# david-jk/BigGAN-Tensorflow

Hardware: AMD Instinct MI355X
Metric: BigGAN-128 train-step images/sec (higher is better)
Workload: dtype bf16; 1 GPU; BigGAN-128 ch=96 bf16 (BASELINE config 3: global batch 256, 32/GPU over 8 GPUs); img_size=128, ch=96, per_gpu_batch=256, global_batch=256, da_policy=full, g_regularization=ortho_cosine, n_labels=0, gan_type=hinge, hip_graph=False, precision=bf16, parallelism=dp1

## Files before the change

### biggan-tensorflow_amd/csrc/igemm16.hip

```cpp
#include <stdlib.h>

#include "common.h"
#include "igemm.h"
#include "igemm16.h"
#include <type_traits>
#include "igemm_dev.h"

namespace bg {

typedef float f32x4_t __attribute__((ext_vector_type(4)));
typedef float f32x16_t __attribute__((ext_vector_type(16)));
typedef __bf16 bf16x8_t __attribute__((ext_vector_type(8)));
typedef short s16x4v __attribute__((ext_vector_type(4)));
typedef short s16x8v __attribute__((ext_vector_type(8)));
typedef __attribute__((address_space(3))) void lds_void_t;
typedef __attribute__((address_space(1))) const void gbl_void_t;
typedef __attribute__((address_space(3))) s16x4v lds_s16x4v;

__device__ uint4 g_zero_page[1024];

__device__ __forceinline__ void glds16(const void* src, unsigned char* lds_wave_base) {
    __builtin_amdgcn_global_load_lds((gbl_void_t*)src, (lds_void_t*)lds_wave_base, 16, 0, 0);
}

__device__ __forceinline__ void glds16_asm(const void* src, uint32_t lds_byte_addr) {
    unsigned keep;
    const uint32_t dst = __builtin_amdgcn_readfirstlane(lds_byte_addr);
    asm volatile("s_mov_b32 %0, m0\n\ts_mov_b32 m0, %2\n\ts_nop 0\n\tglobal_load_lds_dwordx4 %1, off\n\ts_mov_b32 m0, %0"
                 : "=&s"(keep)
                 : "v"(src), "s"(dst)
                 : "memory");
}

__device__ __forceinline__ uint32_t pack_bf16x2(float a, float b) {
    typedef __bf16 bf16x2_t __attribute__((ext_vector_type(2)));
    bf16x2_t v;
    v[0] = (__bf16)a;
    v[1] = (__bf16)b;
    return __builtin_bit_cast(uint32_t, v);
}
__device__ __forceinline__ float bf16_lo(uint32_t u) { return __builtin_bit_cast(float, u << 16); }
__device__ __forceinline__ float bf16_hi(uint32_t u) { return __builtin_bit_cast(float, u & 0xffff0000u); }

constexpr int NN16_BM = 128;
constexpr int NN16_TAPS = 4;
constexpr int NN16_RING_TAPS = 8;
constexpr int nn16_lds_bytes(int TN, int TAPS = NN16_TAPS) {
    const int stage = (NN16_BM + 32 * TN) * 128;
    const int epi = NN16_BM * (32 * TN + 4) * 4;
    const int tab = 2 * TAPS * NN16_BM * 4;
    return (2 * stage + tab > epi ? 2 * stage + tab : epi) + NN16_BM * 4 + 16;
}
constexpr int NN16_NOSRC = -(1 << 30);

template <int MODE>
__device__ __forceinline__ int64_t nn16_src_off(const Gather& g, const RowPos& r, int kh, int kw) {
    int h, w;
    if (MODE == GATHER_CONV) {
        h = conv_src(r.ho, kh, g.stride, g.pad, g.reflect, g.Hs);
        w = conv_src(r.wo, kw, g.stride, g.pad, g.reflect, g.Ws);
    } else {
        h = tconv_src_from_num(r.ho + g.pad - kh, g.stride, g.Hs);
        w = tconv_src_from_num(r.wo + g.pad - kw, g.stride, g.Ws);
    }
    const bool ok = r.valid && h >= 0 && w >= 0;
    const int pix = (r.b * g.Hs + h) * g.Ws + w;
    return ok ? (int64_t)pix * g.ld : (int64_t)-1;
}

constexpr int NN16_NOMIRROR = -(1 << 20);
__device__ __forceinline__ int nn16_mirror_pos(int o, int n, bool hi) {
    return o == 1 ? -1 : ((hi && o == n - 2) ? n : NN16_NOMIRROR);
}

template <int MODE, bool PM, bool RING = false>
__device__ __forceinline__ RowPos nn16_row(const NN16Params& p, int m, int ph, int pw) {
    RowPos r;
    if (PM) {
        r.valid = m < p.M;
        const int pos = m / p.g.Nb;
        r.b = m - pos * p.g.Nb;
        if (RING) {
            const int L = p.ring_lines, first = L * p.g.Wo;
            if (pos < first) {
                const int line = pos / p.g.Wo;
                r.ho = line == 0 ? 1 : p.g.Ho - 2;
                r.wo = pos - line * p.g.Wo;
            } else {
                const int per = p.g.Ho - L, q = pos - first;
                const int line = q / per, idx = q - line * per;
                r.wo = line == 0 ? 1 : p.g.Wo - 2;
                r.ho = idx == 0 ? 0 : ((L == 2 && idx > p.g.Ho - 4) ? p.g.Ho - 1 : idx + 1);
            }
            return r;
        }
        const int hq = pos / p.g.Wq;
        r.ho = hq * p.g.pstep + ph;
        r.wo = (pos - hq * p.g.Wq) * p.g.pstep + pw;
        return r;
    }
    if (MODE == GATHER_PLAIN || !p.pow2) return decompose_row<MODE>(p.g, m, p.M, ph, pw);
    r.valid = m < p.M;
    const int wq = m & (p.g.Wq - 1);
    const int t = m >> p.wq_shift;
    const int hq = t & (p.g.Hq - 1);
    r.b = t >> p.hq_shift;
    r.ho = hq * p.g.pstep + ph;
    r.wo = wq * p.g.pstep + pw;
    return r;
}

template <int TN, int MODE, bool PM, bool RING = false>
__global__ __launch_bounds__(256, 2) void nn16_kernel(const NN16Params p) {
    static_assert(!RING || (PM && MODE == GATHER_TCONV), "ring launches are position-major transposed gathers");
    constexpr int TAPS = RING ? NN16_RING_TAPS : NN16_TAPS;
    constexpr int LDS_BYTES = nn16_lds_bytes(TN, TAPS);
    typedef typename std::conditional<RING, uint64_t, unsigned>::type mask_t;
    constexpr int BM = NN16_BM, BN = 32 * TN;
    constexpr int JA = BM / 32, JB = BN / 32;
    constexpr int A_BYTES = BM * 128, STAGE = (BM + BN) * 128;
    extern __shared__ __attribute__((aligned(16))) unsigned char smem[];

    const int t = threadIdx.x;
    const int lane = t & 63, w = t >> 6;
    const int wm = w >> 1, wn = w & 1;
    const Gather& g = p.g;

    int tile_m, tile_n, bz = blockIdx.z;
    if (p.zfold > 0) {
        const int lin = xcd_remap(blockIdx.x, p.tiles_m * p.tiles_n * p.zfold);
        if (p.mfast) {
            tile_m = lin % p.tiles_m;
            const int r_ = lin / p.tiles_m;
            bz = r_ % p.zfold;
            tile_n = r_ / p.zfold;
        } else {
            bz = lin % p.zfold;
            const int tile = lin / p.zfold;
            tile_n = tile % p.tiles_n;
            tile_m = tile / p.tiles_n;
        }
    } else {
        const int tile = xcd_remap(blockIdx.x, p.tiles_m * p.tiles_n);
        if (p.mfast) {
            tile_m = tile % p.tiles_m;
            tile_n = tile / p.tiles_m;
        } else {
            tile_n = tile % p.tiles_n;
            tile_m = tile / p.tiles_n;
        }
    }
    const int m0 = tile_m * BM, n0 = tile_n * BN;
    const int zs = bz % p.splitk, zo = bz / p.splitk;

    int ph = 0, pw = 0;
    if (MODE == GATHER_TCONV) {
        ph = g.pstep - 1 - zo / g.pstep;
        pw = g.pstep - 1 - zo % g.pstep;
    }
    int kh0 = 0, kw0 = 0, kstep = 1, nkh = g.k, nkw = g.k;
    if (MODE == GATHER_TCONV && g.pstep > 1) {
        kstep = g.stride;
        kh0 = (ph + g.pad) % g.stride;
        kw0 = (pw + g.pad) % g.stride;
        nkh = (g.k - kh0 + g.stride - 1) / g.stride;
        nkw = (g.k - kw0 + g.stride - 1) / g.stride;
    }
    int nrh = 0, nrw = 0;
    if (RING) {
        nrh = nrw = g.k;
        nkh = nkw = 2 * g.k;
    }
    const int C8 = p.C >> 3;
    const int ntap = nkh * nkw;

    unsigned& s_any = *reinterpret_cast<unsigned*>(smem + LDS_BYTES - 16);
    if (PM) {
        if (t == 0) s_any = 0;
        __syncthreads();
    }
    unsigned any_local = 0;
    int* tabh = reinterpret_cast<int*>(smem + 2 * STAGE);
    int* tabw = tabh + TAPS * BM;
    for (int e = t; e < 2 * TAPS * BM; e += 256) {
        const int axis = e / (TAPS * BM), i = (e / BM) % TAPS, row = e % BM;
        const RowPos r = nn16_row<MODE, PM, RING>(p, m0 + row, ph, pw);
        int v = NN16_NOSRC;
        if (r.valid && i < (axis ? nkw : nkh)) {
            int kk = (axis ? kw0 : kh0) + i * kstep;
            int o = axis ? r.wo : r.ho;
            const int n = axis ? g.Ws : g.Hs;
            if (RING) {
                const int nr = axis ? nrw : nrh;
                if (i >= nr) {
                    kk = i - nr;
                    o = nn16_mirror_pos(o, axis ? g.Wo : g.Ho, p.ring_lines == 2);
                }
            }
            const int src = MODE == GATHER_CONV ? conv_src(o, kk, g.stride, g.pad, g.reflect, n)
                                                : (o == NN16_NOMIRROR ? -1 : tconv_src_from_num(o + g.pad - kk, g.stride, n));
            if (src >= 0) {
                v = axis ? src : (r.b * g.Hs + src) * g.Ws;
                any_local |= 1u << (axis * TAPS + i);
            }
        }
        tabh[e] = v;
    }
    if (PM && any_local) atomicOr(&s_any, any_local);
    unsigned* tabo = reinterpret_cast<unsigned*>(smem + LDS_BYTES - 16 - BM * 4);
    constexpr bool use_tabo = MODE == GATHER_TCONV || PM;
    if (use_tabo && t < BM) {
        const RowPos r = nn16_row<MODE, PM, RING>(p, m0 + t, ph, pw);
        tabo[t] = (r.valid && r.ho < g.Ho && r.wo < g.Wo) ? (unsigned)((r.b * g.Ho + r.ho) * g.Wo + r.wo) : 0xffffffffu;
    }

    const int cch = (lane & 7) ^ ((((w & 1) << 2) | (lane >> 4)) & 7);
    const int rsub = 8 * w + (lane >> 3);
    const unsigned char* abase = reinterpret_cast<const unsigned char*>(p.A);
    const unsigned char* bbase = reinterpret_cast<const unsigned char*>(p.B);
    const unsigned char* zero = reinterpret_cast<const unsigned char*>(g_zero_page);
    const unsigned ald2 = 2u * (unsigned)g.ld;
    const uint32_t lds0 = static_cast<uint32_t>(
        reinterpret_cast<uintptr_t>((__attribute__((address_space(3))) unsigned char*)smem));

    __syncthreads();
    mask_t tapmask = 0;
    if (PM) {
        const unsigned any = __builtin_amdgcn_readfirstlane(s_any);
        for (int i = 0; i < nkh; ++i)
            for (int j = 0; j < nkw; ++j)
                if (((any >> i) & (any >> (TAPS + j)) & 1u) != 0 && !(RING && i < nrh && j < nrw))
                    tapmask |= (mask_t)1 << (i * TAPS + j);
    }
    const int nsteps_all = ((PM ? __builtin_popcountll((uint64_t)tapmask) : ntap) * C8 + 7) >> 3;
    const int sps = (nsteps_all + p.splitk - 1) / p.splitk;
    const int it0 = zs * sps;
    const int nsteps = max(0, min(nsteps_all, it0 + sps) - it0);

    mask_t rem = tapmask;
    int tidx = 0, c8, ih = 0, iw = 0;
    {
        const int kk = it0 * 8 + cch;
        tidx = kk / C8;
        c8 = kk - tidx * C8;
        if (PM) {
            for (int i = 0; i < tidx && rem; ++i) rem &= rem - 1;
        } else {
            ih = tidx / nkw;
            iw = tidx - ih * nkw;
        }
    }
    const unsigned char* asrc[JA];
    const unsigned char* wsrc[JB];
    auto set_tap = [&]() {
        bool kvalid;
        if (PM) {
            kvalid = rem != 0;
            const int bit = kvalid ? __builtin_ctzll((uint64_t)rem) : 0;
            ih = bit / TAPS;
            iw = bit % TAPS;
        } else {
            kvalid = tidx < ntap;
        }
        const int* th = tabh + (ih & (TAPS - 1)) * BM + rsub;
        const int* tw = tabw + (iw & (TAPS - 1)) * BM + rsub;
#pragma unroll
        for (int j = 0; j < JA; ++j) {
            const int pix = th[32 * j] + tw[32 * j];
            asrc[j] = (kvalid & (pix >= 0)) ? abase + (uint64_t)(unsigned)pix * ald2 : zero;
        }
        const int kh = RING ? (ih >= nrh ? ih - nrh : ih) : kh0 + ih * kstep;
        const int kw = RING ? (iw >= nrw ? iw - nrw : iw) : kw0 + iw * kstep;
        const unsigned char* wt = bbase + 2 * (int64_t)(kh * g.k + kw) * p.tap_stride;
#pragma unroll
        for (int j = 0; j < JB; ++j) {
            const int n = n0 + 32 * j + rsub;
            wsrc[j] = (kvalid & (n < p.N)) ? wt + 2 * (uint64_t)((unsigned)n * (unsigned)p.C) : zero;
        }
    };
    set_tap();

    auto stage = [&](int buf) {
        const uint32_t sa = lds0 + buf * STAGE + (8 * w) * 128;
        const uint32_t sb = sa + A_BYTES;
        const unsigned cbyte = 16u * (unsigned)c8;
#pragma unroll
        for (int j = 0; j < JA; ++j) glds16_asm(asrc[j] + cbyte, sa + j * 32 * 128);
#pragma unroll
        for (int j = 0; j < JB; ++j) glds16_asm(wsrc[j] + cbyte, sb + j * 32 * 128);
        c8 += 8;
        if (c8 >= C8) {
            do {
                c8 -= C8;
                if (PM) {
                    rem &= rem - 1;
                } else {
                    ++tidx;
                    if (++iw == nkw) {
                        iw = 0;
                        ++ih;
                    }
                }
            } while (c8 >= C8);
            set_tap();
        }
    };

    f32x4_t acc[4][TN];
#pragma unroll
    for (int i = 0; i < 4; ++i)
#pragma unroll
        for (int j = 0; j < TN; ++j)
#pragma unroll
            for (int r = 0; r < 4; ++r) acc[i][j][r] = 0.f;

    const int fsw = (lane & 15) >> 1;
    const int a_row = (wm * 64 + (lane & 15)) * 128;
    const int b_row = A_BYTES + (wn * 16 * TN + (lane & 15)) * 128;
    int koff[2];
#pragma unroll
    for (int s2 = 0; s2 < 2; ++s2) koff[s2] = 16 * ((4 * s2 + (lane >> 4)) ^ fsw);

    if (nsteps > 0) stage(0);
    asm volatile("s_waitcnt vmcnt(0) lgkmcnt(0)" ::: "memory");
    __builtin_amdgcn_s_barrier();

    for (int it = 0; it < nsteps; ++it) {
        const int cur = it & 1;
        if (it + 1 < nsteps) stage(cur ^ 1);
        const unsigned char* sbuf = smem + cur * STAGE;
        bf16x8_t a[2][4], b[2][TN];
#pragma unroll
        for (int s2 = 0; s2 < 2; ++s2) {
#pragma unroll
            for (int i = 0; i < 4; ++i)
                a[s2][i] = *reinterpret_cast<const bf16x8_t*>(sbuf + a_row + i * 16 * 128 + koff[s2]);
#pragma unroll
            for (int j = 0; j < TN; ++j)
                b[s2][j] = *reinterpret_cast<const bf16x8_t*>(sbuf + b_row + j * 16 * 128 + koff[s2]);
        }
#pragma unroll
        for (int s2 = 0; s2 < 2; ++s2)
#pragma unroll
            for (int i = 0; i < 4; ++i)
#pragma unroll
                for (int j = 0; j < TN; ++j)
                    acc[i][j] = __builtin_amdgcn_mfma_f32_16x16x32_bf16(b[s2][j], a[s2][i], acc[i][j], 0, 0, 0);
        asm volatile("s_waitcnt vmcnt(0) lgkmcnt(0)" ::: "memory");
        __builtin_amdgcn_s_barrier();
    }

    constexpr int ELD = BN + 4;
    float* est = reinterpret_cast<float*>(smem);
    const bool partial = p.splitk > 1;
    const float alpha = (!partial && p.alpha) ? *p.alpha : 1.0f;
#pragma unroll
    for (int i = 0; i < 4; ++i)
#pragma unroll
        for (int j = 0; j < TN; ++j) {
            const int row = wm * 64 + 16 * i + (lane & 15);
            const int col = wn * 16 * TN + 16 * j + 4 * (lane >> 4);
            f32x4_t v = acc[i][j];
            v[0] *= alpha; v[1] *= alpha; v[2] *= alpha; v[3] *= alpha;
            *reinterpret_cast<f32x4_t*>(est + row * ELD + col) = v;
        }
    __syncthreads();
    constexpr int CPR = BN / 8;
    float* slab = partial ? p.slabs + (int64_t)zs * p.slab_stride : nullptr;
#pragma unroll
    for (int q = 0; q < BM * CPR / 256; ++q) {
        const int idx = t + 256 * q;
        const int row = idx / CPR, cc = idx - row * CPR;
        const int m = m0 + row, col = n0 + cc * 8;
        if (m >= p.M || col >= p.N) continue;
        int64_t ooff;
        if (use_tabo) {
            const unsigned op = tabo[row];
            if (op == 0xffffffffu) continue;
            ooff = (int64_t)op * p.out_ld + col;
        } else if (p.d2s_c) {
            int b, ho, wo;
            if (p.pow2) {
                wo = m & (g.Wo - 1);
                const int t2 = m >> p.wq_shift;
                ho = t2 & (g.Ho - 1);
                b = t2 >> p.hq_shift;
            } else {
                const int t2 = m / g.Wo;
                wo = m - t2 * g.Wo;
                b = t2 / g.Ho;
                ho = t2 - b * g.Ho;
            }
            const int sub = col / p.d2s_c, c = col - sub * p.d2s_c;
            ooff = (((int64_t)b * (2 * g.Ho) + 2 * ho + (sub >> 1)) * (2 * g.Wo) + 2 * wo + (sub & 1)) * p.d2s_c + c;
        } else {
            ooff = (int64_t)m * p.out_ld + col;
        }
        f32x4_t v0 = *reinterpret_cast<const f32x4_t*>(est + row * ELD + cc * 8);
        f32x4_t v1 = *reinterpret_cast<const f32x4_t*>(est + row * ELD + cc * 8 + 4);
        if (partial) {
            *reinterpret_cast<f32x4_t*>(slab + ooff) = v0;
            *reinterpret_cast<f32x4_t*>(slab + ooff + 4) = v1;
            continue;
        }
        if (p.bias) {
            const f32x4_t b0 = *reinterpret_cast<const f32x4_t*>(p.bias + col);
            const f32x4_t b1 = *reinterpret_cast<const f32x4_t*>(p.bias + col + 4);
            v0 += b0;
            v1 += b1;
        }
        if (p.out_f32) {
            float* o = reinterpret_cast<float*>(p.out) + ooff;
            if (p.accumulate) {
                v0 += *reinterpret_cast<const f32x4_t*>(o);
                v1 += *reinterpret_cast<const f32x4_t*>(o + 4);
            }
            *reinterpret_cast<f32x4_t*>(o) = v0;
            *reinterpret_cast<f32x4_t*>(o + 4) = v1;
        } else {
            __bf16* o = reinterpret_cast<__bf16*>(p.out) + ooff;
            if (p.accumulate) {
                const uint4 r = *reinterpret_cast<const uint4*>(o);
                v0[0] += bf16_lo(r.x); v0[1] += bf16_hi(r.x); v0[2] += bf16_lo(r.y); v0[3] += bf16_hi(r.y);
                v1[0] += bf16_lo(r.z); v1[1] += bf16_hi(r.z); v1[2] += bf16_lo(r.w); v1[3] += bf16_hi(r.w);
            }
            uint4 r;
            r.x = pack_bf16x2(v0[0], v0[1]);
            r.y = pack_bf16x2(v0[2], v0[3]);
            r.z = pack_bf16x2(v1[0], v1[1]);
            r.w = pack_bf16x2(v1[2], v1[3]);
            *reinterpret_cast<uint4*>(o) = r;
        }
    }
}

__global__ __launch_bounds__(256) void nn16_slab_reduce_kernel(const float* __restrict__ slabs, void* __restrict__ out,
                                                               const float* __restrict__ bias,
                                                               const float* __restrict__ alpha_dev, int64_t n8, int N,
                                                               int splitk, int64_t slab_stride, int accumulate,
                                                               int out_f32) {
    const float alpha = alpha_dev ? *alpha_dev : 1.0f;
    for (int64_t i = (int64_t)blockIdx.x * 256 + threadIdx.x; i < n8; i += (int64_t)gridDim.x * 256) {
        f32x4_t s0 = {0.f, 0.f, 0.f, 0.f}, s1 = s0;
        for (int z = 0; z < splitk; ++z) {
            const float* sp = slabs + (int64_t)z * slab_stride + i * 8;
            s0 += *reinterpret_cast<const f32x4_t*>(sp);
            s1 += *reinterpret_cast<const f32x4_t*>(sp + 4);
        }
        s0 *= alpha;
        s1 *= alpha;
        if (bias) {
            const int col = (int)((i * 8) % N);
            s0 += *reinterpret_cast<const f32x4_t*>(bias + col);
            s1 += *reinterpret_cast<const f32x4_t*>(bias + col + 4);
        }
        if (out_f32) {
            float* o = reinterpret_cast<float*>(out) + i * 8;
            if (accumulate) {
                s0 += *reinterpret_cast<const f32x4_t*>(o);
                s1 += *reinterpret_cast<const f32x4_t*>(o + 4);
            }
            *reinterpret_cast<f32x4_t*>(o) = s0;
            *reinterpret_cast<f32x4_t*>(o + 4) = s1;
        } else {
            __bf16* o = reinterpret_cast<__bf16*>(out) + i * 8;
            if (accumulate) {
                const uint4 r = *reinterpret_cast<const uint4*>(o);
                s0[0] += bf16_lo(r.x); s0[1] += bf16_hi(r.x); s0[2] += bf16_lo(r.y); s0[3] += bf16_hi(r.y);
                s1[0] += bf16_lo(r.z); s1[1] += bf16_hi(r.z); s1[2] += bf16_lo(r.w); s1[3] += bf16_hi(r.w);
            }
            uint4 r;
            r.x = pack_bf16x2(s0[0], s0[1]);
            r.y = pack_bf16x2(s0[2], s0[3]);
            r.z = pack_bf16x2(s1[0], s1[1]);
            r.w = pack_bf16x2(s1[2], s1[3]);
            *reinterpret_cast<uint4*>(o) = r;
        }
    }
}

constexpr int NH_T = 16;
constexpr int NH_LDS_MAX = 81920;
template <int NT> struct NHGeom {
    static constexpr int HW = NH_T + NT - 1;
    static constexpr int NPIX = HW * HW;
    static constexpr int A_ROUNDS = (NPIX * 8 + 63) / 64;
    static constexpr int A_INSTR = (A_ROUNDS + 7) / 8;
    static constexpr int A_BYTES = A_ROUNDS * 1024;
};
constexpr int nh_w_rounds(int NF) { return 32 * NF * 8 / 64; }
constexpr int nh_w_instr(int NF) { return (nh_w_rounds(NF) + 7) / 8; }
constexpr int NH_WS = 2;
template <int NT, int NF> constexpr int nn16h_lds_bytes() {
    const int ring = NHGeom<NT>::A_BYTES + NH_WS * nh_w_rounds(NF) * 1024;
    const int epi = 128 * (32 * NF + 4) * 4;
    return ring > epi ? ring : epi;
}

struct NHTile {
    int b, y0, x0, n0, ph, pw, phase, nph, tx, ty, tiles_x, tiles_y;
};
template <int NF, int THIN>
__device__ __forceinline__ void nn16h_epilogue(const NN16Params& p, const NHTile& tl, f32x4_t (&acc)[4][NF],
                                               unsigned char* smem) {
    constexpr int BN = 32 * NF;
    const Gather& g = p.g;
    const int t = threadIdx.x, lane = t & 63, w = t >> 6;
    const int wm = w >> 1, wn = w & 1;
    const int px = lane & 15, kb = lane >> 4;
    const int b = tl.b, y0 = tl.y0, x0 = tl.x0, n0 = tl.n0, ph = tl.ph, pw = tl.pw, phase = tl.phase, nph = tl.nph;
    const int tx = tl.tx, ty = tl.ty, tiles_x = tl.tiles_x, tiles_y = tl.tiles_y;
    constexpr int ELD = BN + 4;
    float* est = reinterpret_cast<float*>(smem);
    const float alpha = p.alpha ? *p.alpha : 1.0f;
    constexpr int CPR = BN / 8;
// ... 761 lines not shown
}

struct NN16Plan {
    int tn, splitk;
};

static int nn16_steps_min(const NN16Params& p, int mode) {
    int per_axis = p.g.k;
    if (mode == GATHER_TCONV && p.g.pstep > 1) per_axis = max(1, p.g.k / p.g.stride);
    return (per_axis * per_axis * (p.C >> 3) + 7) >> 3;
}

static double nn16_axis_fraction(const Gather& g, int mode, int nq, int n_src) {
    int64_t valid = 0, slots = 0;
    for (int ph = 0; ph < (mode == GATHER_TCONV ? g.pstep : 1); ++ph) {
        int k0 = 0, kstep = 1, nk = g.k;
        if (mode == GATHER_TCONV && g.pstep > 1) {
            kstep = g.stride;
            k0 = (ph + g.pad) % g.stride;
            nk = (g.k - k0 + g.stride - 1) / g.stride;
        }
        for (int q = 0; q < nq; ++q) {
            const int o = q * g.pstep + ph;
            for (int i = 0; i < nk; ++i) {
                const int kk = k0 + i * kstep;
                bool ok;
                if (mode == GATHER_CONV) {
                    const int src = o * g.stride + kk - g.pad;
                    ok = g.reflect || (src >= 0 && src < n_src);
                } else {
                    const int hn = o + g.pad - kk;
                    ok = hn >= 0 && hn % g.stride == 0 && hn / g.stride < n_src;
                }
                valid += ok;
            }
            slots += nk;
        }
    }
    return slots ? (double)valid / (double)slots : 1.0;
}

static double nn16_posmajor_fraction(const NN16Params& p, int mode) {
    const char* e = getenv("BG_NN16_POSMAJOR");
    if (e && atoi(e) == 0) return 1.0;
    const Gather& g = p.g;
    if (g.k <= 1 || g.Nb < 16 || g.Hq <= 0 || g.Wq <= 0 || (int64_t)g.Hq * g.Wq > 40 * 40) return 1.0;
    const double f = nn16_axis_fraction(g, mode, g.Hq, g.Hs) * nn16_axis_fraction(g, mode, g.Wq, g.Ws);
    return f < 0.9 ? f : 1.0;
}

static NN16Plan plan_nn16(const NN16Params& p, int mode, int zdim, bool allow_split) {
    static const int slots = getenv("BG_NN16_SLOTS") ? atoi(getenv("BG_NN16_SLOTS")) : 512;
    const int64_t tm = (p.M + NN16_BM - 1) / NN16_BM;
    int steps = nn16_steps_min(p, mode);
    const double pm = nn16_posmajor_fraction(p, mode);
    if (pm < 1.0) steps = max(1, (int)(steps * pm + 0.5));
    NN16Plan best{4, 1};
    double best_cost = 1e30;
    for (int tn = 4; tn >= 1; --tn) {
        const int bn = 32 * tn;
        const int64_t tiles = tm * ((p.N + bn - 1) / bn) * zdim;
        const double unit = 1.5 + tn;
        const int max_sk = allow_split ? (steps / 4 < 16 ? (steps / 4 < 1 ? 1 : steps / 4) : 16) : 1;
        for (int sk = 1; sk <= max_sk; ++sk) {
            const int64_t rounds = (tiles * sk + slots - 1) / slots;
            double cost = (double)rounds * ((steps + sk - 1) / sk + 2.0) * unit;
            if (sk > 1) cost += 6.0 * unit + 0.02 * sk * (double)tiles / slots * bn;
            if (cost < best_cost - 1e-9) {
                best_cost = cost;
                best = NN16Plan{tn, sk};
            }
        }
    }
    return best;
}

size_t nn16_workspace_bytes(const NN16Params& p, int mode, int zdim, int64_t out_elems) {
    const NN16Plan pl = plan_nn16(p, mode, zdim, true);
    return pl.splitk > 1 ? (size_t)pl.splitk * out_elems * sizeof(float) : 0;
}

static int nn16_mfast(const NN16Params& p, int tiles_m, int tiles_n);

template <int TN>
static int launch_nn16_ring_inst(const NN16Params& p, dim3 grid, hipStream_t s) {
    constexpr int lds = nn16_lds_bytes(TN, NN16_RING_TAPS);
    if (!lds_opt_in(reinterpret_cast<const void*>(&nn16_kernel<TN, GATHER_TCONV, true, true>), lds)) return BG_ERR_LAUNCH;
    hipLaunchKernelGGL((nn16_kernel<TN, GATHER_TCONV, true, true>), grid, dim3(256), lds, s, p);
    return BG_OK;
}

int launch_nn16_ring(NN16Params& p, hipStream_t s) {
    BG_REQUIRE(p.ring == 1 && (p.ring_lines == 1 || p.ring_lines == 2), "nn16 ring launch: ring = 1, ring_lines 1 or 2");
    BG_REQUIRE(p.g.k >= 1 && p.g.k <= NN16_RING_TAPS / 2 && p.g.Ho >= 4 && p.g.Wo >= 4 && p.accumulate == 1,
               "nn16 ring launch: kernel size %d / map %d x %d not supported", p.g.k, p.g.Ho, p.g.Wo);
    BG_REQUIRE(p.C % 8 == 0 && p.N % 8 == 0 && p.g.ld % 8 == 0 && p.out_ld % 8 == 0, "nn16 ring launch: channels %% 8");
    const int npos = p.ring_lines * p.g.Wo + p.ring_lines * (p.g.Ho - p.ring_lines);
    p.g.pstep = 1;
    p.g.Hq = 1;
    p.g.Wq = npos;
    p.M = p.g.Nb * npos;
    p.posmajor = 1;
    p.splitk = 1;
    p.slabs = nullptr;
    p.zfold = 0;
    p.pow2 = 0;
    int tn = 4, best = 1 << 30;
    for (int c = 4; c >= 1; --c) {
        const int padded = (p.N + 32 * c - 1) / (32 * c) * (32 * c);
        if (padded < best) { best = padded; tn = c; }
    }
    p.tiles_m = (p.M + NN16_BM - 1) / NN16_BM;
    p.tiles_n = (p.N + 32 * tn - 1) / (32 * tn);
    p.mfast = nn16_mfast(p, p.tiles_m, p.tiles_n);
    dim3 grid(p.tiles_m * p.tiles_n, 1, 1);
    int rc;
    switch (tn) {
        case 1: rc = launch_nn16_ring_inst<1>(p, grid, s); break;
        case 2: rc = launch_nn16_ring_inst<2>(p, grid, s); break;
        case 3: rc = launch_nn16_ring_inst<3>(p, grid, s); break;
        default: rc = launch_nn16_ring_inst<4>(p, grid, s); break;
    }
    if (rc) return rc;
    BG_LAUNCH_CHECK();
    return BG_OK;
}

template <int TN, int MODE, bool PM>
static int launch_nn16_inst(const NN16Params& p, dim3 grid, hipStream_t s) {
    constexpr int lds = nn16_lds_bytes(TN);
    if (!lds_opt_in(reinterpret_cast<const void*>(&nn16_kernel<TN, MODE, PM>), lds)) return BG_ERR_LAUNCH;
    prof_kernel("nn16_kernel<%d, %d, %s>", TN, MODE, PM ? "true" : "false");
    hipLaunchKernelGGL((nn16_kernel<TN, MODE, PM>), grid, dim3(256), lds, s, p);
    return BG_OK;
}

template <int MODE, bool PM>
static int launch_nn16_pm(const NN16Params& p, int tn, dim3 grid, hipStream_t s) {
    switch (tn) {
        case 1: return launch_nn16_inst<1, MODE, PM>(p, grid, s);
        case 2: return launch_nn16_inst<2, MODE, PM>(p, grid, s);
        case 3: return launch_nn16_inst<3, MODE, PM>(p, grid, s);
        default: return launch_nn16_inst<4, MODE, PM>(p, grid, s);
    }
}

template <int MODE>
static int launch_nn16_mode(const NN16Params& p, int tn, dim3 grid, hipStream_t s) {
    return p.posmajor ? launch_nn16_pm<MODE, true>(p, tn, grid, s) : launch_nn16_pm<MODE, false>(p, tn, grid, s);
}

static int nn16h_taps(const NN16Params& p, int mode, int zdim) {
    const char* e = getenv("BG_NN16_HALO");
    const int use = e ? atoi(e) : 1;
    static const int cmax = getenv("BG_NN16_HALO_CMAX") ? atoi(getenv("BG_NN16_HALO_CMAX")) : 4096;
    const Gather& g = p.g;
    if (!use || p.C > cmax || p.C % 32 || p.N % 8 || g.Hq < NH_T || g.Wq < NH_T || g.Hq % NH_T || g.Wq % NH_T) return 0;
    if (mode == GATHER_CONV) return (g.stride == 1 && g.k == 3 && g.pstep == 1 && zdim == 1) ? 3 : 0;
    if (g.reflect) return 0;
    if (g.stride == 1 && g.k == 3 && g.pstep == 1 && zdim == 1) return 3;
    if (g.stride == 2 && g.k == 4 && g.pstep == 2 && zdim == 4) return 2;
    if (g.stride == 2 && g.k == 3 && g.pad == 1 && g.pstep == 2 && zdim == 4) {
        const char* e3 = getenv("BG_NN16_HALO_K3S2");
        return (e3 && atoi(e3) == 1) ? 2 : 0;
    }
    return 0;
}

template <int NT, int NF, int MODE, int THIN = 0>
static int launch_nn16h_inst(const NN16Params& p, int blocks, hipStream_t s) {
    constexpr int lds = nn16h_lds_bytes<NT, NF>();
    if (!lds_opt_in(reinterpret_cast<const void*>(&nn16h_kernel<NT, NF, MODE, THIN>), lds)) return BG_ERR_LAUNCH;
    if (THIN) prof_kernel("nn16h_kernel<%d, %d, %d, d2s>", NT, NF, MODE);
    else prof_kernel("nn16h_kernel<%d, %d, %d>", NT, NF, MODE);
    hipLaunchKernelGGL((nn16h_kernel<NT, NF, MODE, THIN>), dim3(blocks), dim3(512), lds, s, p);
    return BG_OK;
}

template <int NT, int MODE>
static int launch_nn16h_nf(const NN16Params& p, int nf, int blocks, hipStream_t s) {
    switch (nf) {
        case 1: return launch_nn16h_inst<NT, 1, MODE>(p, blocks, s);
        case 2: return launch_nn16h_inst<NT, 2, MODE>(p, blocks, s);
        case 3: return launch_nn16h_inst<NT, 3, MODE>(p, blocks, s);
        default: return launch_nn16h_inst<NT, 4, MODE>(p, blocks, s);
    }
}

bool nn16h_d2s_ok(const NN16Params& p) {
    const char* e = getenv("BG_THIN_D2S");
    const int use = e ? atoi(e) : 1;
    const Gather& g = p.g;
    return use && p.N == 8 && p.out_ld == 8 && g.k == 3 && g.stride == 2 && g.pad == 1 && !g.reflect && p.C % 32 == 0 &&
           g.Hs % NH_T == 0 && g.Ws % NH_T == 0 && g.Ho == 2 * g.Hs && g.Wo == 2 * g.Ws && !p.bias && !p.stats_part;
}
int launch_nn16h_d2s(const NN16Params& plain, hipStream_t s) {
    BG_REQUIRE(nn16h_d2s_ok(plain), "nn16h depth-to-space form: unsupported geometry");
    NN16Params p = plain;
    Gather& g = p.g;
    g.Hq = g.Hs; g.Wq = g.Ws; g.pstep = 1; g.pad = 0; g.stride = 1;
    p.N = 32;
    p.splitk = 1; p.mfast = 0; p.ring = 0;
    const int64_t blocks = (int64_t)g.Nb * (g.Hq / NH_T) * (g.Wq / NH_T);
    BG_REQUIRE(blocks > 0 && blocks < (int64_t(1) << 31), "nn16h: grid out of range");
    if (const int rc = launch_nn16h_inst<2, 1, GATHER_CONV, 1>(p, (int)blocks, s)) return rc;
    BG_LAUNCH_CHECK();
    return BG_OK;
}

static int nn16_mfast(const NN16Params& p, int tiles_m, int tiles_n) {
    const char* e = getenv("BG_NN16_MFAST");
    if (!e) return 0;
    if (strcmp(e, "auto") != 0) return atoi(e) != 0;
    const double l2 = 3.0e6;
    const double a_bytes = 2.0 * p.g.Nb * (double)p.g.Hs * p.g.Ws * p.g.ld;
    const double w_bytes = 2.0 * p.g.k * p.g.k * (double)p.N * p.C;
    const double nfast = a_bytes + (w_bytes > l2 ? w_bytes * tiles_m : w_bytes);
    const double mfast = w_bytes + (a_bytes > l2 ? a_bytes * tiles_n : a_bytes);
    return mfast < nfast;
}

static int launch_nn16h(NN16Params& p, int mode, int ntaps, hipStream_t s) {
    int nf = 4, best = 1 << 30;
    for (int c = 4; c >= 1; --c) {
        const int padded = (p.N + 32 * c - 1) / (32 * c) * (32 * c);
        if (padded < best) { best = padded; nf = c; }
    }
    const Gather& g = p.g;
    const int64_t blocks = (int64_t)g.Nb * (g.Hq / NH_T) * (g.Wq / NH_T) * ((p.N + 32 * nf - 1) / (32 * nf)) *
                           (g.pstep * g.pstep);
    BG_REQUIRE(blocks > 0 && blocks < (int64_t(1) << 31), "nn16h: grid out of range");
    p.splitk = 1;
    p.mfast = nn16_mfast(p, g.Nb * (g.Hq / NH_T) * (g.Wq / NH_T), (p.N + 32 * nf - 1) / (32 * nf));
    int rc;
    if (mode == GATHER_CONV) rc = launch_nn16h_nf<3, GATHER_CONV>(p, nf, (int)blocks, s);
    else if (ntaps == 3) rc = launch_nn16h_nf<3, GATHER_TCONV>(p, nf, (int)blocks, s);
    else rc = launch_nn16h_nf<2, GATHER_TCONV>(p, nf, (int)blocks, s);
    if (rc) return rc;
    BG_LAUNCH_CHECK();
    return BG_OK;
}

bool nn16_d2s_ok(const NN16Params& p, int mode, int zdim) {
    const Gather& g = p.g;
    if (p.d2s_c <= 0 || p.d2s_c % 8 || p.N != 4 * p.d2s_c || p.C % 8 || mode != GATHER_CONV || zdim != 1 || g.stride != 1 ||
        g.pstep != 1 || g.Hq != g.Ho || g.Wq != g.Wo || p.stats_part || p.ring)
        return false;
    if ((int64_t)g.Nb * g.Ho * g.Wo * 4 >= (int64_t(1) << 31)) return false;
    if (nn16h_taps(p, mode, zdim)) return true;
    if (nn16_posmajor_fraction(p, mode) < 1.0) return false;
    return plan_nn16(p, mode, zdim, true).splitk == 1;
}

int64_t nn16_stats_rows(const NN16Params& p, int mode, int zdim) {
    if (p.C % 8 || p.N % 8 || !nn16h_taps(p, mode, zdim)) return 0;
    return 2 * (int64_t)p.g.Nb * (p.g.Hq / NH_T) * (p.g.Wq / NH_T) * (p.g.pstep * p.g.pstep);
}

int launch_nn16(NN16Params& p, int mode, int zdim, int64_t out_elems, void* ws, size_t ws_bytes, hipStream_t s) {
    BG_REQUIRE(p.C % 8 == 0 && p.N % 8 == 0 && p.g.ld % 8 == 0 && p.out_ld % 8 == 0,
               "bf16-resident conv: channel counts must be multiples of 8 (C=%d N=%d)", p.C, p.N);
    BG_REQUIRE((reinterpret_cast<uintptr_t>(p.A) & 15) == 0 && (reinterpret_cast<uintptr_t>(p.B) & 15) == 0 &&
                   (reinterpret_cast<uintptr_t>(p.out) & 15) == 0,
               "bf16-resident conv: tensors must be 16-byte aligned");
    BG_REQUIRE(p.g.k >= 1 && p.g.k <= NN16_TAPS && p.C <= 8192 && p.g.stride >= 1 && p.g.stride <= 2,
               "bf16-resident conv: kernel size %d / stride %d / %d channels not supported", p.g.k, p.g.stride, p.C);
    BG_REQUIRE((int64_t)p.g.Nb * p.g.Hs * p.g.Ws < (int64_t(1) << 30) && (int64_t)p.g.Nb * p.g.Ho * p.g.Wo < (int64_t(1) << 31),
               "bf16-resident conv: more than 2^30 source / 2^31 output pixels");
    BG_REQUIRE(p.d2s_c == 0 || (nn16_d2s_ok(p, mode, zdim) && ws == nullptr),
               "bf16-resident conv: this launch has no depth-to-space store (bg_conv2d_fwd_d2s_supported)");
    if (const int ntaps = nn16h_taps(p, mode, zdim)) return launch_nn16h(p, mode, ntaps, s);
    BG_REQUIRE(p.stats_part == nullptr, "bf16-resident conv: fused statistics need the halo-tile form (nn16_stats_rows)");
    NN16Plan pl = plan_nn16(p, mode, zdim, ws != nullptr);
    if (pl.splitk > 1 && ws_bytes < (size_t)pl.splitk * out_elems * sizeof(float)) pl.splitk = 1;
    p.splitk = pl.splitk;
    p.slabs = reinterpret_cast<float*>(ws);
    p.slab_stride = out_elems;
    const int bn = 32 * pl.tn;
    p.tiles_m = (p.M + NN16_BM - 1) / NN16_BM;
    p.tiles_n = (p.N + bn - 1) / bn;
    p.pow2 = 0;
    if (p.g.Wq > 0 && p.g.Hq > 0 && (p.g.Wq & (p.g.Wq - 1)) == 0 && (p.g.Hq & (p.g.Hq - 1)) == 0) {
        p.pow2 = 1;
        p.wq_shift = __builtin_ctz(p.g.Wq);
        p.hq_shift = __builtin_ctz(p.g.Hq);
    }
    p.posmajor = nn16_posmajor_fraction(p, mode) < 1.0;
    p.mfast = nn16_mfast(p, p.tiles_m, p.tiles_n);
    dim3 grid(p.tiles_m * p.tiles_n, 1, zdim * p.splitk);
    p.zfold = 0;
    if (mode == GATHER_TCONV && zdim > 1 && p.splitk == 1 && p.g.k % p.g.stride == 0) {
        p.zfold = zdim;
        grid = dim3(p.tiles_m * p.tiles_n * zdim, 1, 1);
    }
    int rc;
    if (mode == GATHER_CONV)
        rc = launch_nn16_mode<GATHER_CONV>(p, pl.tn, grid, s);
    else
        rc = launch_nn16_mode<GATHER_TCONV>(p, pl.tn, grid, s);
    if (rc) return rc;
    BG_LAUNCH_CHECK();
    if (pl.splitk > 1) {
        const int64_t n8 = out_elems / 8;
        int blocks = (int)((n8 + 255) / 256);
        if (blocks > 2048) blocks = 2048;
        hipLaunchKernelGGL(nn16_slab_reduce_kernel, dim3(blocks), dim3(256), 0, s, p.slabs, p.out, p.bias, p.alpha, n8,
                           p.N, pl.splitk, out_elems, p.accumulate, p.out_f32);
        BG_LAUNCH_CHECK();
    }
    return BG_OK;
}

static void plan_tn16(TN16Params& p) {
    const int64_t tiles = (int64_t)((p.Mf + 127) / 128) * ((p.Cb + 127) / 128);
    static const int want = getenv("BG_TN16_WANT") ? atoi(getenv("BG_TN16_WANT")) : 1024;
    int sk = (int)(want / tiles);
    const int max_sk = (p.M + 4 * TN16_BK - 1) / (4 * TN16_BK);
    if (sk > max_sk) sk = max_sk;
    if (sk < 1) sk = 1;
    if (sk > 512) sk = 512;
    int rps = (p.M + sk - 1) / sk;
    rps = (rps + TN16_BK - 1) / TN16_BK * TN16_BK;
    p.splitk = (p.M + rps - 1) / rps;
    p.rows_per_split = rps;
}

static int tn16x_nbi(const TN16Params& p) {
    const char* e = getenv("BG_TN16X_NBI");
    if (!e || atoi(e) != 2) return 1;
    return (p.Cb >= 512 && p.Cb % 256 == 0 && p.Mf >= 256) ? 2 : 1;
}

static bool plan_tn16x(const TN16Params& p, int* sk_out, int* rps_out) {
    static const int use_wide = getenv("BG_TN16_WIDE") ? atoi(getenv("BG_TN16_WIDE")) : 1;
    if (!use_wide || p.Mf <= 128 || p.M < 8 * TN16_BK) return false;
    if (p.g.k > 0 && (p.g.Wq <= 0 || p.g.Hq <= 0 || (p.g.Wq & (p.g.Wq - 1)) || (p.g.Hq & (p.g.Hq - 1)))) return false;
    const int nbi = tn16x_nbi(p);
    const int tm = (p.Mf + 255) / 256, tn = (p.Cb + 128 * nbi - 1) / (128 * nbi);
    static const int wantx0 = getenv("BG_TN16X_WANT") ? atoi(getenv("BG_TN16X_WANT")) : 512;
    const int wantx = nbi == 2 ? wantx0 / 2 : wantx0;
    int sk = wantx / (tm * tn);
    const int max_sk = (p.M + 4 * TN16_BK - 1) / (4 * TN16_BK);
    if (sk > max_sk) sk = max_sk;
    if (sk < 1) sk = 1;
    if (sk > 512) sk = 512;
    int rps = (p.M + sk - 1) / sk;
    rps = (rps + TN16_BK - 1) / TN16_BK * TN16_BK;
    *sk_out = (p.M + rps - 1) / rps;
    *rps_out = rps;
    return true;
}

size_t tn16_workspace_bytes(const TN16Params& p0) {
    TN16Params p = p0;
    plan_tn16(p);
    int sk = p.splitk, skx = 1, rps = 0;
    if (plan_tn16x(p0, &skx, &rps) && skx > sk) sk = skx;
    return sk > 1 ? (size_t)sk * p.Mf * p.Cb * sizeof(float) : 0;
}

int launch_tn16(TN16Params& p, int mode, float* final_out, void* ws, size_t ws_bytes, hipStream_t s) {
    BG_REQUIRE(p.Ca % 8 == 0 && p.Cb % 8 == 0 && p.g.ld % 8 == 0 && p.b_ld % 8 == 0,
               "bf16-resident wgrad: channel counts must be multiples of 8 (Ca=%d Cb=%d)", p.Ca, p.Cb);
    BG_REQUIRE((reinterpret_cast<uintptr_t>(p.A) & 15) == 0 && (reinterpret_cast<uintptr_t>(p.Bv) & 15) == 0,
               "bf16-resident wgrad: tensors must be 16-byte aligned");
    plan_tn16(p);
    const int64_t total = (int64_t)p.Mf * p.Cb;
    if (p.splitk > 1 && (ws == nullptr || ws_bytes < (size_t)p.splitk * total * sizeof(float) || p.out_ld != p.Cb)) {
        p.splitk = 1;
        p.rows_per_split = (p.M + TN16_BK - 1) / TN16_BK * TN16_BK;
    }
    if (p.splitk > 1) {
        p.out = reinterpret_cast<float*>(ws);
        p.slab_stride = total;
    } else {
        p.out = final_out;
        p.slab_stride = 0;
    }
    p.tiles_m = (p.Mf + 127) / 128;
    p.tiles_n = (p.Cb + 127) / 128;
    p.pow2 = 0;
    if (mode != GATHER_PLAIN && (p.g.Wq & (p.g.Wq - 1)) == 0 && (p.g.Hq & (p.g.Hq - 1)) == 0) {
// ... 77 lines not shown
```

Measured before the change: 2673 images/sec.

## Add 3-slot LDS ring pipeline and 8-wave wide-tile form to nn16 conv

Adds a pipelined variant of the bf16 implicit-GEMM conv kernel. It uses a 3-slot LDS ring with half-width K steps (4 chunks), int16 column tables, and a partitioned epilogue, so loads for step k+2 overlap the MFMAs of step k. A wide 256-row, 8-wave form is chosen by default for small-channel, non-position-major launches with enough blocks, while the ring form is opt-in via an environment variable. The aim is better latency hiding and occupancy, at the cost of more barriers per K and changed tile shapes.

Result: faster. 2720 images/sec, median of 6 (+1.8%).

```diff
diff --git a/biggan-tensorflow_amd/csrc/igemm16.hip b/biggan-tensorflow_amd/csrc/igemm16.hip
--- a/biggan-tensorflow_amd/csrc/igemm16.hip
+++ b/biggan-tensorflow_amd/csrc/igemm16.hip
@@ -50,6 +50,10 @@
     const int epi = NN16_BM * (32 * TN + 4) * 4;
     const int tab = 2 * TAPS * NN16_BM * 4;
     return (2 * stage + tab > epi ? 2 * stage + tab : epi) + NN16_BM * 4 + 16;
+}
+constexpr int nn16_pipe_lds_bytes(int TN, int WM, int TAPS = NN16_TAPS) {
+    const int bm = 64 * WM;
+    return 3 * (bm + 32 * TN) * 64 + TAPS * bm * (4 + 2) + bm * 4 + 16;
 }
 constexpr int NN16_NOSRC = -(1 << 30);
 
@@ -110,19 +114,31 @@
     return r;
 }
 
-template <int TN, int MODE, bool PM, bool RING = false>
-__global__ __launch_bounds__(256, 2) void nn16_kernel(const NN16Params p) {
+template <int TN, int MODE, bool PM, bool RING = false, int SLOTS = 2, int WM = 2>
+__global__ __launch_bounds__(128 * WM, SLOTS == 2 ? 2 : (WM == 4 ? 4 : 3)) void nn16_kernel(const NN16Params p) {
     static_assert(!RING || (PM && MODE == GATHER_TCONV), "ring launches are position-major transposed gathers");
+    static_assert((SLOTS == 2 && WM == 2) || (SLOTS == 3 && (WM == 2 || WM == 4)), "two stages, or a 3-slot ring on 4 / 8 waves");
+    constexpr bool PIPE = SLOTS == 3;
     constexpr int TAPS = RING ? NN16_RING_TAPS : NN16_TAPS;
-    constexpr int LDS_BYTES = nn16_lds_bytes(TN, TAPS);
+    constexpr int LDS_BYTES = PIPE ? nn16_pipe_lds_bytes(TN, WM, TAPS) : nn16_lds_bytes(TN, TAPS);
     typedef typename std::conditional<RING, uint64_t, unsigned>::type mask_t;
-    constexpr int BM = NN16_BM, BN = 32 * TN;
-    constexpr int JA = BM / 32, JB = BN / 32;
-    constexpr int A_BYTES = BM * 128, STAGE = (BM + BN) * 128;
+    typedef typename std::conditional<PIPE, int16_t, int>::type tabw_t;
+    constexpr int BM = 64 * WM, BN = 32 * TN, NTHR = 128 * WM, NWV = 2 * WM;
+    constexpr int CPS = PIPE ? 4 : 8;
+    constexpr int ROWB = 16 * CPS;
+    constexpr int RSTR = PIPE ? 16 * NWV : 32;
+    constexpr int JA = BM / RSTR, JB = PIPE ? (BN / 16 + NWV - 1) / NWV : BN / 32;
+    constexpr int A_BYTES = BM * ROWB, STAGE = (BM + BN) * ROWB;
+    static_assert(BM == NN16_BM || PIPE, "the two-stage form has 128-row tiles");
+    static_assert(A_BYTES % 1024 == 0 && STAGE % 1024 == 0 && (RSTR * ROWB) % 1024 == 0,
+                  "every LDS-DMA destination is 1 KB aligned");
+    static_assert(!PIPE || 64 * (BN + 4) * 4 <= SLOTS * STAGE, "a 64-row part of the epilogue fits in front of the tables");
+    static_assert(!PIPE || RING || LDS_BYTES * (WM == 4 ? 2 : 3) <= 160 * 1024, "ring forms: 3 (8 waves: 2) blocks per CU");
+    static_assert(!PIPE || LDS_BYTES * 2 <= 160 * 1024, "mirrored-tap ring launches: 2 blocks per CU");
     extern __shared__ __attribute__((aligned(16))) unsigned char smem[];
 
     const int t = threadIdx.x;
-    const int lane = t & 63, w = t >> 6;
+    const int lane = t & 63, w = PIPE ? __builtin_amdgcn_readfirstlane(t >> 6) : t >> 6;
     const int wm = w >> 1, wn = w & 1;
     const Gather& g = p.g;
 
@@ -180,9 +196,9 @@
         __syncthreads();
     }
     unsigned any_local = 0;
-    int* tabh = reinterpret_cast<int*>(smem + 2 * STAGE);
-    int* tabw = tabh + TAPS * BM;
-    for (int e = t; e < 2 * TAPS * BM; e += 256) {
+    int* tabh = reinterpret_cast<int*>(smem + SLOTS * STAGE);
+    tabw_t* tabw = reinterpret_cast<tabw_t*>(tabh + TAPS * BM);
+    for (int e = t; e < 2 * TAPS * BM; e += NTHR) {
         const int axis = e / (TAPS * BM), i = (e / BM) % TAPS, row = e % BM;
         const RowPos r = nn16_row<MODE, PM, RING>(p, m0 + row, ph, pw);
         int v = NN16_NOSRC;
@@ -204,7 +220,8 @@
                 any_local |= 1u << (axis * TAPS + i);
             }
         }
-        tabh[e] = v;
+        if (PIPE && axis) tabw[e - TAPS * BM] = (tabw_t)(v < 0 ? -1 : v);
+        else tabh[e] = v;
     }
     if (PM && any_local) atomicOr(&s_any, any_local);
     unsigned* tabo = reinterpret_cast<unsigned*>(smem + LDS_BYTES - 16 - BM * 4);
@@ -214,8 +231,10 @@
         tabo[t] = (r.valid && r.ho < g.Ho && r.wo < g.Wo) ? (unsigned)((r.b * g.Ho + r.ho) * g.Wo + r.wo) : 0xffffffffu;
     }
 
-    const int cch = (lane & 7) ^ ((((w & 1) << 2) | (lane >> 4)) & 7);
-    const int rsub = 8 * w + (lane >> 3);
+    const int cch = PIPE ? (lane & 3) ^ ((lane >> 3) & 2) : (lane & 7) ^ ((((w & 1) << 2) | (lane >> 4)) & 7);
+    const int rsub = PIPE ? 16 * w + (lane >> 2) : 8 * w + (lane >> 3);
+    constexpr int NB_HI = JB, NB_LO = (BN / 16) / NWV;
+    const int nbw = (PIPE && NB_HI != NB_LO) ? (BN / 16 - w + NWV - 1) / NWV : JB;
     const unsigned char* abase = reinterpret_cast<const unsigned char*>(p.A);
     const unsigned char* bbase = reinterpret_cast<const unsigned char*>(p.B);
     const unsigned char* zero = reinterpret_cast<const unsigned char*>(g_zero_page);
@@ -263,10 +282,12 @@
             kvalid = tidx < ntap;
         }
         const int* th = tabh + (ih & (TAPS - 1)) * BM + rsub;
-        const int* tw = tabw + (iw & (TAPS - 1)) * BM + rsub;
+        const tabw_t* tw = tabw + (iw & (TAPS - 1)) * BM + rsub;
 #pragma unroll
         for (int j = 0; j < JA; ++j) {
-            const int pix = th[32 * j] + tw[32 * j];
+            int col = tw[RSTR * j];
+            if (PIPE) col = col < 0 ? NN16_NOSRC : col;
+            const int pix = th[RSTR * j] + col;
             asrc[j] = (kvalid & (pix >= 0)) ? abase + (uint64_t)(unsigned)pix * ald2 : zero;
         }
         const int kh = RING ? (ih >= nrh ? ih - nrh : ih) : kh0 + ih * kstep;
@@ -274,21 +295,13 @@
         const unsigned char* wt = bbase + 2 * (int64_t)(kh * g.k + kw) * p.tap_stride;
 #pragma unroll
         for (int j = 0; j < JB; ++j) {
-            const int n = n0 + 32 * j + rsub;
+            const int n = n0 + RSTR * j + rsub;
             wsrc[j] = (kvalid & (n < p.N)) ? wt + 2 * (uint64_t)((unsigned)n * (unsigned)p.C) : zero;
         }
     };
     set_tap();
-
-    auto stage = [&](int buf) {
-        const uint32_t sa = lds0 + buf * STAGE + (8 * w) * 128;
-        const uint32_t sb = sa + A_BYTES;
-        const unsigned cbyte = 16u * (unsigned)c8;
-#pragma unroll
-        for (int j = 0; j < JA; ++j) glds16_asm(asrc[j] + cbyte, sa + j * 32 * 128);
-#pragma unroll
-        for (int j = 0; j < JB; ++j) glds16_asm(wsrc[j] + cbyte, sb + j * 32 * 128);
-        c8 += 8;
+    auto advance = [&]() {
+        c8 += CPS;
         if (c8 >= C8) {
             do {
                 c8 -= C8;
@@ -306,6 +319,18 @@
         }
     };
 
+    auto stage = [&](int buf) {
+        const uint32_t sa = lds0 + buf * STAGE + w * 1024;
+        const uint32_t sb = sa + A_BYTES;
+        const unsigned cbyte = 16u * (unsigned)c8;
+#pragma unroll
+        for (int j = 0; j < JA; ++j) glds16_asm(asrc[j] + cbyte, sa + j * RSTR * ROWB);
+#pragma unroll
+        for (int j = 0; j < JB; ++j)
+            if (!PIPE || j < nbw) glds16_asm(wsrc[j] + cbyte, sb + j * RSTR * ROWB);
+        advance();
+    };
+
     f32x4_t acc[4][TN];
 #pragma unroll
     for (int i = 0; i < 4; ++i)
@@ -314,6 +339,40 @@
 #pragma unroll
             for (int r = 0; r < 4; ++r) acc[i][j][r] = 0.f;
 
+    if constexpr (PIPE) {
+        const int frag = (lane & 15) * ROWB + 16 * ((lane >> 4) ^ (((lane & 15) >> 1) & 2));
+        const unsigned char* a_ad = smem + wm * 64 * ROWB + frag;
+        const unsigned char* b_ad = smem + A_BYTES + wn * 16 * TN * ROWB + frag;
+        const int nst = 2 * nsteps;
+        if (nst > 0) stage(0);
+        if (nst > 1) stage(1);
+        auto kstep = [&](int it, auto slot_c) {
+            constexpr int SLOT = decltype(slot_c)::value;
+            if (it + 1 < nst) {
+                if (NB_HI == NB_LO || nbw == NB_HI) asm volatile("s_waitcnt vmcnt(%0) lgkmcnt(0)" ::"n"(JA + NB_HI) : "memory");
+                else asm volatile("s_waitcnt vmcnt(%0) lgkmcnt(0)" ::"n"(JA + NB_LO) : "memory");
+            } else
+                asm volatile("s_waitcnt vmcnt(0) lgkmcnt(0)" ::: "memory");
+            __builtin_amdgcn_s_barrier();
+            if (it + 2 < nst) stage((SLOT + 2) % 3);
+            bf16x8_t a[4], b[TN];
+#pragma unroll
+            for (int i = 0; i < 4; ++i) a[i] = *reinterpret_cast<const bf16x8_t*>(a_ad + SLOT * STAGE + i * 16 * ROWB);
+#pragma unroll
+            for (int j = 0; j < TN; ++j) b[j] = *reinterpret_cast<const bf16x8_t*>(b_ad + SLOT * STAGE + j * 16 * ROWB);
+#pragma unroll
+            for (int i = 0; i < 4; ++i)
+#pragma unroll
+                for (int j = 0; j < TN; ++j)
+                    acc[i][j] = __builtin_amdgcn_mfma_f32_16x16x32_bf16(b[j], a[i], acc[i][j], 0, 0, 0);
+        };
+        for (int it = 0; it < nst; it += 3) {
+            kstep(it, std::integral_constant<int, 0>());
+            if (it + 1 < nst) kstep(it + 1, std::integral_constant<int, 1>());
+            if (it + 2 < nst) kstep(it + 2, std::integral_constant<int, 2>());
+        }
+        __syncthreads();
+    } else {
     const int fsw = (lane & 15) >> 1;
     const int a_row = (wm * 64 + (lane & 15)) * 128;
     const int b_row = A_BYTES + (wn * 16 * TN + (lane & 15)) * 128;
@@ -349,28 +408,37 @@
         asm volatile("s_waitcnt vmcnt(0) lgkmcnt(0)" ::: "memory");
         __builtin_amdgcn_s_barrier();
     }
-
+    }
+
+    constexpr int PARTS = PIPE ? WM : 1, PR = BM / PARTS;
     constexpr int ELD = BN + 4;
     float* est = reinterpret_cast<float*>(smem);
     const bool partial = p.splitk > 1;
     const float alpha = (!partial && p.alpha) ? *p.alpha : 1.0f;
-#pragma unroll
-    for (int i = 0; i < 4; ++i)
-#pragma unroll
-        for (int j = 0; j < TN; ++j) {
-            const int row = wm * 64 + 16 * i + (lane & 15);
-            const int col = wn * 16 * TN + 16 * j + 4 * (lane >> 4);
-            f32x4_t v = acc[i][j];
-            v[0] *= alpha; v[1] *= alpha; v[2] *= alpha; v[3] *= alpha;
-            *reinterpret_cast<f32x4_t*>(est + row * ELD + col) = v;
-        }
-    __syncthreads();
     constexpr int CPR = BN / 8;
     float* slab = partial ? p.slabs + (int64_t)zs * p.slab_stride : nullptr;
 #pragma unroll
-    for (int q = 0; q < BM * CPR / 256; ++q) {
-        const int idx = t + 256 * q;
-        const int row = idx / CPR, cc = idx - row * CPR;
+    for (int part = 0; part < PARTS; ++part) {
+    if (part > 0) __syncthreads();
+    if (!PIPE || wm == part) {
+#pragma unroll
+        for (int i = 0; i < 4; ++i)
+#pragma unroll
+            for (int j = 0; j < TN; ++j) {
+                const int row = (PIPE ? 0 : wm * 64) + 16 * i + (lane & 15);
+                const int col = wn * 16 * TN + 16 * j + 4 * (lane >> 4);
+                f32x4_t v = acc[i][j];
+                v[0] *= alpha; v[1] *= alpha; v[2] *= alpha; v[3] *= alpha;
+                *reinterpret_cast<f32x4_t*>(est + row * ELD + col) = v;
+            }
+    }
+    __syncthreads();
+#pragma unroll
+    for (int q = 0; q < (PR * CPR + NTHR - 1) / NTHR; ++q) {
+        const int idx = t + NTHR * q;
+        if ((PR * CPR) % NTHR != 0 && idx >= PR * CPR) continue;
+        const int erow = idx / CPR, cc = idx - erow * CPR;
+        const int row = part * PR + erow;
         const int m = m0 + row, col = n0 + cc * 8;
         if (m >= p.M || col >= p.N) continue;
         int64_t ooff;
@@ -396,8 +464,8 @@
         } else {
             ooff = (int64_t)m * p.out_ld + col;
         }
-        f32x4_t v0 = *reinterpret_cast<const f32x4_t*>(est + row * ELD + cc * 8);
-        f32x4_t v1 = *reinterpret_cast<const f32x4_t*>(est + row * ELD + cc * 8 + 4);
+        f32x4_t v0 = *reinterpret_cast<const f32x4_t*>(est + erow * ELD + cc * 8);
+        f32x4_t v1 = *reinterpret_cast<const f32x4_t*>(est + erow * ELD + cc * 8 + 4);
         if (partial) {
             *reinterpret_cast<f32x4_t*>(slab + ooff) = v0;
             *reinterpret_cast<f32x4_t*>(slab + ooff + 4) = v1;
@@ -431,6 +499,7 @@
             r.w = pack_bf16x2(v1[2], v1[3]);
             *reinterpret_cast<uint4*>(o) = r;
         }
+    }
     }
 }
 
@@ -1358,12 +1427,28 @@
 
 static int nn16_mfast(const NN16Params& p, int tiles_m, int tiles_n);
 
+enum { NN16_FORM_TWO = 0, NN16_FORM_RING = 1, NN16_FORM_WIDE = 2 };
+static int nn16_form(const NN16Params& p, int tn, int64_t wide_blocks, bool mirrored) {
+    if (p.g.Ws >= (1 << 15)) return NN16_FORM_TWO;
+    const bool wide_ok = !mirrored && !p.posmajor;
+    if (const char* e = getenv("BG_NN16_PIPE")) {
+        const int v = atoi(e);
+        if (v == 2) return wide_ok ? NN16_FORM_WIDE : NN16_FORM_TWO;
+        return v == 1 ? NN16_FORM_RING : NN16_FORM_TWO;
+    }
+    return (wide_ok && p.C <= 192 && tn >= 2 && wide_blocks >= 512) ? NN16_FORM_WIDE : NN16_FORM_TWO;
+}
+
+template <int TN, int SLOTS = 2>
+static int launch_nn16_ring_inst(const NN16Params& p, dim3 grid, hipStream_t s) {
+    constexpr int lds = SLOTS == 3 ? nn16_pipe_lds_bytes(TN, 2, NN16_RING_TAPS) : nn16_lds_bytes(TN, NN16_RING_TAPS);
+    if (!lds_opt_in(reinterpret_cast<const void*>(&nn16_kernel<TN, GATHER_TCONV, true, true, SLOTS>), lds)) return BG_ERR_LAUNCH;
+    hipLaunchKernelGGL((nn16_kernel<TN, GATHER_TCONV, true, true, SLOTS>), grid, dim3(256), lds, s, p);
+    return BG_OK;
+}
 template <int TN>
-static int launch_nn16_ring_inst(const NN16Params& p, dim3 grid, hipStream_t s) {
-    constexpr int lds = nn16_lds_bytes(TN, NN16_RING_TAPS);
-    if (!lds_opt_in(reinterpret_cast<const void*>(&nn16_kernel<TN, GATHER_TCONV, true, true>), lds)) return BG_ERR_LAUNCH;
-    hipLaunchKernelGGL((nn16_kernel<TN, GATHER_TCONV, true, true>), grid, dim3(256), lds, s, p);
-    return BG_OK;
+static int launch_nn16_ring_tn(const NN16Params& p, int form, dim3 grid, hipStream_t s) {
+    return form == NN16_FORM_RING ? launch_nn16_ring_inst<TN, 3>(p, grid, s) : launch_nn16_ring_inst<TN>(p, grid, s);
 }
 
 int launch_nn16_ring(NN16Params& p, hipStream_t s) {
@@ -1390,40 +1475,50 @@
     p.tiles_n = (p.N + 32 * tn - 1) / (32 * tn);
     p.mfast = nn16_mfast(p, p.tiles_m, p.tiles_n);
     dim3 grid(p.tiles_m * p.tiles_n, 1, 1);
+    const int form = nn16_form(p, tn, 0, true);
     int rc;
     switch (tn) {
-        case 1: rc = launch_nn16_ring_inst<1>(p, grid, s); break;
-        case 2: rc = launch_nn16_ring_inst<2>(p, grid, s); break;
-        case 3: rc = launch_nn16_ring_inst<3>(p, grid, s); break;
-        default: rc = launch_nn16_ring_inst<4>(p, grid, s); break;
+        case 1: rc = launch_nn16_ring_tn<1>(p, form, grid, s); break;
+        case 2: rc = launch_nn16_ring_tn<2>(p, form, grid, s); break;
+        case 3: rc = launch_nn16_ring_tn<3>(p, form, grid, s); break;
+        default: rc = launch_nn16_ring_tn<4>(p, form, grid, s); break;
     }
     if (rc) return rc;
     BG_LAUNCH_CHECK();
     return BG_OK;
 }
 
+template <int TN, int MODE, bool PM, int SLOTS = 2, int WM = 2>
+static int launch_nn16_inst(const NN16Params& p, dim3 grid, hipStream_t s) {
+    constexpr int lds = SLOTS == 3 ? nn16_pipe_lds_bytes(TN, WM) : nn16_lds_bytes(TN);
+    if (!lds_opt_in(reinterpret_cast<const void*>(&nn16_kernel<TN, MODE, PM, false, SLOTS, WM>), lds)) return BG_ERR_LAUNCH;
+    if (SLOTS == 2) prof_kernel("nn16_kernel<%d, %d, %s>", TN, MODE, PM ? "true" : "false");
+    else prof_kernel("nn16_kernel<%d, %d, %s, false, %d, %d>", TN, MODE, PM ? "true" : "false", SLOTS, WM);
+    hipLaunchKernelGGL((nn16_kernel<TN, MODE, PM, false, SLOTS, WM>), grid, dim3(128 * WM), lds, s, p);
+    return BG_OK;
+}
+
 template <int TN, int MODE, bool PM>
-static int launch_nn16_inst(const NN16Params& p, dim3 grid, hipStream_t s) {
-    constexpr int lds = nn16_lds_bytes(TN);
-    if (!lds_opt_in(reinterpret_cast<const void*>(&nn16_kernel<TN, MODE, PM>), lds)) return BG_ERR_LAUNCH;
-    prof_kernel("nn16_kernel<%d, %d, %s>", TN, MODE, PM ? "true" : "false");
-    hipLaunchKernelGGL((nn16_kernel<TN, MODE, PM>), grid, dim3(256), lds, s, p);
-    return BG_OK;
+static int launch_nn16_tn(const NN16Params& p, int form, dim3 grid, hipStream_t s) {
+    if (form == NN16_FORM_RING) return launch_nn16_inst<TN, MODE, PM, 3, 2>(p, grid, s);
+    if constexpr (!PM)
+        if (form == NN16_FORM_WIDE) return launch_nn16_inst<TN, MODE, PM, 3, 4>(p, grid, s);
+    return launch_nn16_inst<TN, MODE, PM>(p, grid, s);
 }
 
 template <int MODE, bool PM>
-static int launch_nn16_pm(const NN16Params& p, int tn, dim3 grid, hipStream_t s) {
+static int launch_nn16_pm(const NN16Params& p, int tn, int form, dim3 grid, hipStream_t s) {
     switch (tn) {
-        case 1: return launch_nn16_inst<1, MODE, PM>(p, grid, s);
-        case 2: return launch_nn16_inst<2, MODE, PM>(p, grid, s);
-        case 3: return launch_nn16_inst<3, MODE, PM>(p, grid, s);
-        default: return launch_nn16_inst<4, MODE, PM>(p, grid, s);
+        case 1: return launch_nn16_tn<1, MODE, PM>(p, form, grid, s);
+        case 2: return launch_nn16_tn<2, MODE, PM>(p, form, grid, s);
+        case 3: return launch_nn16_tn<3, MODE, PM>(p, form, grid, s);
+        default: return launch_nn16_tn<4, MODE, PM>(p, form, grid, s);
     }
 }
 
 template <int MODE>
-static int launch_nn16_mode(const NN16Params& p, int tn, dim3 grid, hipStream_t s) {
-    return p.posmajor ? launch_nn16_pm<MODE, true>(p, tn, grid, s) : launch_nn16_pm<MODE, false>(p, tn, grid, s);
+static int launch_nn16_mode(const NN16Params& p, int tn, int form, dim3 grid, hipStream_t s) {
+    return p.posmajor ? launch_nn16_pm<MODE, true>(p, tn, form, grid, s) : launch_nn16_pm<MODE, false>(p, tn, form, grid, s);
 }
 
 static int nn16h_taps(const NN16Params& p, int mode, int zdim) {
@@ -1553,15 +1648,17 @@
     p.slabs = reinterpret_cast<float*>(ws);
     p.slab_stride = out_elems;
     const int bn = 32 * pl.tn;
-    p.tiles_m = (p.M + NN16_BM - 1) / NN16_BM;
     p.tiles_n = (p.N + bn - 1) / bn;
+    p.posmajor = nn16_posmajor_fraction(p, mode) < 1.0;
+    const int form = nn16_form(p, pl.tn, (int64_t)((p.M + 255) / 256) * p.tiles_n * zdim * pl.splitk, false);
+    const int bm = form == NN16_FORM_WIDE ? 256 : NN16_BM;
+    p.tiles_m = (p.M + bm - 1) / bm;
     p.pow2 = 0;
     if (p.g.Wq > 0 && p.g.Hq > 0 && (p.g.Wq & (p.g.Wq - 1)) == 0 && (p.g.Hq & (p.g.Hq - 1)) == 0) {
         p.pow2 = 1;
         p.wq_shift = __builtin_ctz(p.g.Wq);
         p.hq_shift = __builtin_ctz(p.g.Hq);
     }
-    p.posmajor = nn16_posmajor_fraction(p, mode) < 1.0;
     p.mfast = nn16_mfast(p, p.tiles_m, p.tiles_n);
     dim3 grid(p.tiles_m * p.tiles_n, 1, zdim * p.splitk);
     p.zfold = 0;
@@ -1571,9 +1668,9 @@
     }
     int rc;
     if (mode == GATHER_CONV)
-        rc = launch_nn16_mode<GATHER_CONV>(p, pl.tn, grid, s);
+        rc = launch_nn16_mode<GATHER_CONV>(p, pl.tn, form, grid, s);
     else
-        rc = launch_nn16_mode<GATHER_TCONV>(p, pl.tn, grid, s);
+        rc = launch_nn16_mode<GATHER_TCONV>(p, pl.tn, form, grid, s);
     if (rc) return rc;
     BG_LAUNCH_CHECK();
     if (pl.splitk > 1) {
```
